# HoundThe/yara

Measured on AMD Instinct MI355X. Metric: scanned GB/s per GPU (4 GiB buffer, 10k atoms) + bit-exact match-set vs CPU, higher is better.
Workload: dtype u8; 1 GPU; config C: 10000 strings -> AC tables of stock libyara 4.2.1, 4 GiB per GPU; bytes_per_gpu=4294967296, parallelism=shard1

## Files before the change

include/yara_amd.h:

```cpp
#ifndef YARA_AMD_H
#define YARA_AMD_H

#include <stddef.h>
#include <stdint.h>

#ifdef __cplusplus
extern "C" {
#endif

#define YR_AMD_SUCCESS                0
#define YR_AMD_INSUFFICIENT_MEMORY    1
#define YR_AMD_COULD_NOT_MAP_FILE     4
#define YR_AMD_SCAN_TIMEOUT          26
#define YR_AMD_CALLBACK_ERROR        28
#define YR_AMD_INVALID_ARGUMENT      29
#define YR_AMD_INTERNAL_FATAL_ERROR  31

#define YR_AMD_MAX_ATOM_LENGTH 4

typedef struct yr_amd_tables yr_amd_tables;
typedef struct yr_amd_scanner yr_amd_scanner;

int yr_amd_tables_create(
    const uint32_t* transition_table,
// ... 42 lines not shown

int yr_amd_scan_block(
    yr_amd_scanner* scanner,
    const uint8_t* data,
    size_t size,
    const uint64_t** positions,
    uint64_t* count,
    int* all_positions);

int yr_amd_scan_device(
    yr_amd_scanner* scanner,
    const uint8_t* d_data,
    uint64_t block_size,
    uint64_t byte_begin,
    uint64_t byte_end);

int yr_amd_scan_window(
    yr_amd_scanner* scanner,
    const uint8_t* d_window,
    uint64_t window_begin,
    uint64_t window_end,
    uint64_t block_size,
    uint64_t byte_begin,
    uint64_t byte_end);

int yr_amd_scan_device_result(
    yr_amd_scanner* scanner,
    const uint64_t** d_positions,
    uint64_t* count,
    int* all_positions);

int yr_amd_scanner_set_verified_only(yr_amd_scanner* scanner, int enable);

int yr_amd_scan_device_stream_length(yr_amd_scanner* scanner, uint64_t* length);

typedef int (*yr_amd_verify_fn)(void* user, uint32_t pool_index, uint64_t offset);

int yr_amd_replay(
    const yr_amd_tables* tables,
    const uint8_t* data,
    size_t size,
    const uint64_t* positions,
    uint64_t count,
    int all_positions,
    yr_amd_verify_fn verify,
    void* user);

typedef struct
{
  uint64_t position;
  uint32_t state;
  uint32_t match;
} yr_amd_trace_rec;

int yr_amd_trace_walk(
    yr_amd_scanner* scanner,
    const uint8_t* d_data,
    size_t size,
    uint64_t data_base,
    yr_amd_trace_rec* out,
    uint64_t cap,
    uint64_t* count);

typedef struct
{
  uint32_t flags;
// ... 237 lines not shown
```

yara_amd/__init__.py:

```python
import ctypes

import numpy as np

from . import _lib
from ._lib import (CALLBACK_ERROR, COULD_NOT_MAP_FILE, INSUFFICIENT_MEMORY,
                   INTERNAL_FATAL_ERROR, INVALID_ARGUMENT, MATCH_HEX, MATCH_LITERAL,
                   MAX_ATOM_LENGTH, SCAN_TIMEOUT, SUCCESS, YaraAmdError)

__all__ = ["Tables", "Scanner", "Pipeline", "replay", "fill_xorshift64", "version",
           "batch_layout", "merge_matches", "YaraAmdError", "MATCH_LITERAL", "MATCH_HEX"]


def _arr(a, dt):
    return np.ascontiguousarray(a, dtype=dt)


def version() -> str:
    return _lib.lib().yr_amd_version().decode()


def batch_layout(sizes):
    sz = _arr(sizes, np.uint64).reshape(-1)
    st = np.zeros(sz.size, np.uint64)
    arena = ctypes.c_uint64()
# ... 466 lines not shown
    def scan_window(self, d_ptr: int, window_begin: int, window_end: int, block_size: int,
                    byte_begin: int, byte_end: int):
        _lib.check("yr_amd_scan_window",
                   _lib.lib().yr_amd_scan_window(self._h, ctypes.c_void_p(d_ptr), window_begin,
                                                 window_end, block_size, byte_begin, byte_end))

    def device_result(self):
        p = ctypes.c_void_p()
        cnt = ctypes.c_uint64()
        allp = ctypes.c_int()
        _lib.check("yr_amd_scan_device_result",
                   _lib.lib().yr_amd_scan_device_result(self._h, ctypes.byref(p), ctypes.byref(cnt),
                                                        ctypes.byref(allp)))
        return p.value or 0, cnt.value, bool(allp.value)

    def trace_walk(self, d_ptr: int, size: int, data_base: int = 0, cap=None):
        cnt = ctypes.c_uint64()
        if cap is None:
            _lib.check("yr_amd_trace_walk",
                       _lib.lib().yr_amd_trace_walk(self._h, ctypes.c_void_p(d_ptr), size, data_base,
                                                    None, 0, ctypes.byref(cnt)))
            cap = cnt.value
        out = np.zeros(cap, dtype=_lib.TRACE_REC_DTYPE)
        _lib.check("yr_amd_trace_walk",
                   _lib.lib().yr_amd_trace_walk(self._h, ctypes.c_void_p(d_ptr), size, data_base,
                                                ctypes.c_void_p(out.ctypes.data if cap else 0), cap,
                                                ctypes.byref(cnt)))
        return out[:min(cap, cnt.value)], cnt.value

    def set_verified_only(self, enable: bool = True):
        _lib.check("yr_amd_scanner_set_verified_only",
                   _lib.lib().yr_amd_scanner_set_verified_only(self._h, int(enable)))

    def stream_length(self) -> int:
        n = ctypes.c_uint64()
        _lib.check("yr_amd_scan_device_stream_length",
                   _lib.lib().yr_amd_scan_device_stream_length(self._h, ctypes.byref(n)))
        return n.value

    def set_timing(self, enable: bool = True):
        _lib.check("yr_amd_scanner_set_timing", _lib.lib().yr_amd_scanner_set_timing(self._h, int(enable)))

    def kernel_ms(self) -> float:
        ms = ctypes.c_float()
        _lib.check("yr_amd_scanner_kernel_ms", _lib.lib().yr_amd_scanner_kernel_ms(self._h, ctypes.byref(ms)))
        return ms.value

    def scan_ms(self) -> float:
        ms = ctypes.c_float()
        _lib.check("yr_amd_scanner_scan_ms", _lib.lib().yr_amd_scanner_scan_ms(self._h, ctypes.byref(ms)))
        return ms.value

    def close(self):
        if getattr(self, "_h", None):
            _lib.lib().yr_amd_scanner_destroy(self._h)
            self._h = None

    def __del__(self):
        try:
            self.close()
        except Exception:
            pass


def merge_matches(blocks):
    parts = []
# ... 139 lines not shown
```

yara_amd/_lib.py:

```python
import ctypes
import os

_HERE = os.path.dirname(os.path.abspath(__file__))
LIB_PATH = os.environ.get("YARA_AMD_LIB") or os.path.join(_HERE, "libyara_amd.so")

SUCCESS = 0
INSUFFICIENT_MEMORY = 1
COULD_NOT_MAP_FILE = 4
SCAN_TIMEOUT = 26
CALLBACK_ERROR = 28
INVALID_ARGUMENT = 29
INTERNAL_FATAL_ERROR = 31
MAX_ATOM_LENGTH = 4
MATCH_MAX_BLOCK = 1 << 32

_u32p = ctypes.POINTER(ctypes.c_uint32)
_u16p = ctypes.POINTER(ctypes.c_uint16)
_u64p = ctypes.POINTER(ctypes.c_uint64)
_u8p = ctypes.POINTER(ctypes.c_uint8)
_vp = ctypes.c_void_p
_int = ctypes.c_int

VERIFY_FN = ctypes.CFUNCTYPE(ctypes.c_int, ctypes.c_void_p, ctypes.c_uint32, ctypes.c_uint64)
COPY_FN = ctypes.CFUNCTYPE(ctypes.c_int, ctypes.c_void_p, ctypes.c_void_p, ctypes.c_void_p,
# ... 32 lines not shown
class MatchRec(ctypes.Structure):
    _fields_ = [("offset", ctypes.c_uint64), ("string", ctypes.c_uint32),
                ("length", ctypes.c_uint32), ("xor_key", ctypes.c_uint32),
                ("pool_index", ctypes.c_uint32)]


VERIFY_REC_DTYPE = [("offset", "<u8"), ("pool_index", "<u4"), ("candidate", "<u4")]
MATCH_REC_DTYPE = [("offset", "<u8"), ("string", "<u4"), ("length", "<u4"), ("xor_key", "<u4"),
                   ("pool_index", "<u4")]
TRACE_REC_DTYPE = [("position", "<u8"), ("state", "<u4"), ("match", "<u4")]

PROTOTYPES = {
    "yr_amd_tables_create": (_int, [_u32p, _u32p, ctypes.c_uint32, _u32p, _u16p, ctypes.c_uint32,
                                    _int, ctypes.POINTER(_vp)]),
    "yr_amd_tables_destroy": (_int, [_vp]),
    "yr_amd_tables_load_yarc": (_int, [_u8p, ctypes.c_size_t, _int, ctypes.POINTER(_vp)]),
    "yr_amd_tables_get_info": (_int, [_vp, ctypes.POINTER(TablesInfo)]),
    "yr_amd_scanner_create": (_int, [_vp, _vp, ctypes.POINTER(_vp)]),
    "yr_amd_scanner_destroy": (_int, [_vp]),
    "yr_amd_scan_block": (_int, [_vp, _u8p, ctypes.c_size_t, ctypes.POINTER(_u64p),
                                 ctypes.POINTER(ctypes.c_uint64), ctypes.POINTER(_int)]),
    "yr_amd_scan_device": (_int, [_vp, _vp, ctypes.c_uint64, ctypes.c_uint64, ctypes.c_uint64]),
    "yr_amd_scan_window": (_int, [_vp, _vp, ctypes.c_uint64, ctypes.c_uint64, ctypes.c_uint64,
                                  ctypes.c_uint64, ctypes.c_uint64]),
    "yr_amd_scan_device_result": (_int, [_vp, ctypes.POINTER(_vp), ctypes.POINTER(ctypes.c_uint64),
                                         ctypes.POINTER(_int)]),
    "yr_amd_replay": (_int, [_vp, _u8p, ctypes.c_size_t, _u64p, ctypes.c_uint64, _int, VERIFY_FN,
                             _vp]),
    "yr_amd_trace_walk": (_int, [_vp, _vp, ctypes.c_size_t, ctypes.c_uint64, _vp, ctypes.c_uint64,
                                 ctypes.POINTER(ctypes.c_uint64)]),
    "yr_amd_fill_xorshift64": (_int, [_vp, ctypes.c_uint64, ctypes.c_uint64, ctypes.c_uint64, _vp]),
    "yr_amd_scanner_set_timing": (_int, [_vp, _int]),
    "yr_amd_scanner_set_verified_only": (_int, [_vp, _int]),
    "yr_amd_scan_device_stream_length": (_int, [_vp, _u64p]),
    "yr_amd_scanner_kernel_ms": (_int, [_vp, ctypes.POINTER(ctypes.c_float)]),
    "yr_amd_scanner_scan_ms": (_int, [_vp, ctypes.POINTER(ctypes.c_float)]),
    "yr_amd_version": (ctypes.c_char_p, []),
    "yr_amd_tables_set_strings": (_int, [_vp, _u32p, ctypes.c_uint32, ctypes.POINTER(String),
                                         ctypes.c_uint32, _u8p, ctypes.c_uint64, _u8p]),
    "yr_amd_tables_set_re_code": (_int, [_vp, ctypes.c_uint32, _u32p, _u32p, _u32p, _u32p, _u8p,
                                         ctypes.c_uint64]),
    "yr_amd_re_code_extent": (_int, [_u8p, ctypes.c_uint64, ctypes.POINTER(ctypes.c_uint32)]),
    "yr_amd_verify_device": (_int, [_vp, ctypes.c_uint64, ctypes.POINTER(_vp),
                                    ctypes.POINTER(ctypes.c_uint64)]),
    "yr_amd_tables_final_strings": (_int, [_vp, _u8p, ctypes.c_uint32]),
    "yr_amd_tables_set_string_flags": (_int, [_vp, _u32p, ctypes.c_uint32]),
    "yr_amd_tables_string_count": (_int, [_vp, _u32p]),
    "yr_amd_match_device": (_int, [_vp, ctypes.c_uint64, ctypes.POINTER(_vp),
                                   ctypes.POINTER(ctypes.c_uint64), ctypes.POINTER(_vp),
                                   ctypes.POINTER(ctypes.c_uint64)]),
    "yr_amd_scan_block_matches": (_int, [_vp, _u8p, ctypes.c_size_t, ctypes.c_uint64,
                                         ctypes.POINTER(ctypes.POINTER(MatchRec)),
                                         ctypes.POINTER(ctypes.c_uint64),
                                         ctypes.POINTER(ctypes.POINTER(VerifyRec)),
                                         ctypes.POINTER(ctypes.c_uint64)]),
    "yr_amd_pipeline_create": (_int, [_vp, ctypes.c_uint32, ctypes.POINTER(_vp)]),
    "yr_amd_pipeline_destroy": (_int, [_vp]),
    "yr_amd_pipeline_submit": (_int, [_vp, _u8p, ctypes.c_size_t, ctypes.c_uint64]),
    "yr_amd_pipeline_submit_dma": (_int, [_vp, _u8p, ctypes.c_size_t, ctypes.c_uint64]),
    "yr_amd_pipeline_next": (_int, [_vp, ctypes.POINTER(ctypes.POINTER(VerifyRec)),
                                    ctypes.POINTER(ctypes.c_uint64), ctypes.POINTER(_u8p),
                                    ctypes.POINTER(ctypes.c_size_t), ctypes.POINTER(ctypes.c_uint64)]),
    "yr_amd_pipeline_drain": (_int, [_vp]),
    "yr_amd_pipeline_create_multi": (_int, [ctypes.POINTER(_vp), ctypes.c_uint32, ctypes.c_uint32,
                                            ctypes.POINTER(_vp)]),
    "yr_amd_pipeline_set_copy": (_int, [_vp, COPY_FN, _vp]),
# ... 72 lines not shown
```

yara_amd/csrc/internal.h:

```cpp
#pragma once

#include <stdint.h>
#include <stdlib.h>

#include <hip/hip_runtime.h>

#ifndef YAMD_DIAG
#define YAMD_DIAG 0
#endif

namespace yamd {

inline const char* diag_env(const char* name) { return YAMD_DIAG ? getenv(name) : nullptr; }

constexpr int kWave = 64;
constexpr int kBytesPerLane = 16;
constexpr int kTile = kWave * kBytesPerLane;
constexpr uint32_t kSegment = 1u << 20;
constexpr uint32_t kSegmentTarget = kSegment;
constexpr uint32_t kMaxByteKeys = 4;
constexpr uint32_t kMaxPairKeys = 4;
constexpr int kWavesPerWG = 16;
constexpr int kWGThreads = kWave * kWavesPerWG;

constexpr int kFilterLog2Bits = 20;
constexpr uint32_t kFilterWords = 1u << (kFilterLog2Bits - 5);
constexpr uint32_t kFilterBytes = kFilterWords * 4;

constexpr uint32_t kQueueCap = 64;
constexpr uint32_t kQueueEntryWords = 6;
constexpr uint32_t kQueueBytes = kWavesPerWG * kQueueCap * kQueueEntryWords * 4;
constexpr uint32_t kPendBytes = kWavesPerWG * kWave * 8;
constexpr uint32_t kScanLdsBytes = kFilterBytes + kQueueBytes + kPendBytes;

constexpr uint32_t kFilterPair = 0;
constexpr uint32_t kFilterEven = 1;
constexpr uint32_t kFilterEvenHash = 2;
constexpr uint32_t kEvenHashK = 0xEBCA77u;
struct FilterProbe {
  uint32_t block;
  uint32_t b_lo, b_hi;
};
__host__ __device__ inline FilterProbe filter_probe_left(uint32_t w3) {
  const uint32_t x = w3 & 0xFFFFFFu;
  return FilterProbe{x >> 10, x & 31u, (x >> 5) & 31u};
}
__host__ __device__ inline FilterProbe filter_probe_even(uint32_t w3, bool hashed) {
  const uint32_t x = w3 & 0xFFFFFFu;
  const uint32_t block = hashed ? (x * kEvenHashK) >> 18 : x >> 10;
  return FilterProbe{block, x & 31u, (x >> 5) & 31u};
}
__host__ __device__ inline FilterProbe filter_probe_right(uint32_t w3) {
// ... 92 lines not shown
```

yara_amd/csrc/kernels.hip:

```cpp
#include <hip/hip_ext.h>

#include "internal.h"

namespace yamd {

__device__ __forceinline__ uint32_t lane_id() {
  return __builtin_amdgcn_mbcnt_hi(~0u, __builtin_amdgcn_mbcnt_lo(~0u, 0u));
}

typedef uint32_t u32x2 __attribute__((ext_vector_type(2)));
template <typename T>
__device__ __forceinline__ T lds_load(uint32_t addr) {
  return *reinterpret_cast<const __attribute__((address_space(3))) T*>((uintptr_t)addr);
}
__device__ __forceinline__ void lds_store2(uint32_t addr, uint32_t x, uint32_t y) {
  u32x2 v;
  v.x = x;
  v.y = y;
  *reinterpret_cast<__attribute__((address_space(3))) u32x2*>((uintptr_t)addr) = v;
}

__device__ __forceinline__ uint32_t wave_inclusive_scan(uint32_t v) {
  v += __builtin_amdgcn_update_dpp(0u, v, 0x111, 0xF, 0xF, true);
  v += __builtin_amdgcn_update_dpp(0u, v, 0x112, 0xF, 0xF, true);
  v += __builtin_amdgcn_update_dpp(0u, v, 0x114, 0xF, 0xF, true);
  v += __builtin_amdgcn_update_dpp(0u, v, 0x118, 0xF, 0xF, true);
  v += __builtin_amdgcn_update_dpp(0u, v, 0x142, 0xA, 0xF, false);
  v += __builtin_amdgcn_update_dpp(0u, v, 0x143, 0xC, 0xF, false);
  return v;
}

__device__ __forceinline__ bool bucket_pair_has(const uint4& a, const uint4& b, uint32_t k) {
  const uint32_t x = min(min(a.x ^ k, a.y ^ k), a.z ^ k);
// ... 1106 lines not shown
    for (int i = 0; i < YAMD_PAD_VOP2; i += 4)
      asm volatile("v_add_u32_e32 %0, 1, %0\n v_add_u32_e32 %1, 1, %1\n v_add_u32_e32 %2, 1, %2\n v_add_u32_e32 %3, 1, %3"
                   : "+v"(t0), "+v"(t1), "+v"(t2), "+v"(t3));
#endif
#ifdef YAMD_PAD_VOP3
#pragma unroll
    for (int i = 0; i < YAMD_PAD_VOP3; i += 4)
      asm volatile("v_add3_u32 %0, %0, 1, 2\n v_add3_u32 %1, %1, 1, 2\n v_add3_u32 %2, %2, 1, 2\n v_add3_u32 %3, %3, 1, 2"
                   : "+v"(t0), "+v"(t1), "+v"(t2), "+v"(t3));
#endif
#ifdef YAMD_PAD_NOP
#pragma unroll
    for (int i = 0; i < YAMD_PAD_NOP; ++i) asm volatile("s_nop 0");
#endif
    asm volatile("" ::"v"(t0 ^ t1 ^ t2 ^ t3));
#ifdef YAMD_PAD_SALU
    uint32_t u0 = tile_off, u1 = tile_off + 1, u2 = tile_off + 2, u3 = tile_off + 3;
#pragma unroll
    for (int i = 0; i < YAMD_PAD_SALU; i += 4)
      asm volatile("s_add_u32 %0, %0, 1\n s_add_u32 %1, %1, 1\n s_add_u32 %2, %2, 1\n s_add_u32 %3, %3, 1"
                   : "+s"(u0), "+s"(u1), "+s"(u2), "+s"(u3) : : "scc");
    asm volatile("" ::"s"(u0 ^ u1 ^ u2 ^ u3));
#endif
  }
#endif
  if constexpr (kAbl<MODE> == 1) {
    asm volatile("" ::"v"(any));
  } else {
    ring_append<MODE, TAIL>(p, q, st, S, any, tile_off, lane);
  }
  if constexpr (kBkSkipF<MODE>) q.facc |= any_f;
}

template <int MODE>
__device__ __forceinline__ void scan_segment(const ScanParams& p, WaveQueue& q, uint32_t seg, uint32_t lane) {
  SegState st;
  st.seg_start = p.byte_begin + (uint64_t)seg * p.seg_bytes;
  const uint64_t seg_end = min(st.seg_start + p.seg_bytes, p.byte_end);
  st.seg_len = (uint32_t)(seg_end - st.seg_start);
  st.out = p.seg_out + (p.seg_base ? p.seg_base[seg] : (size_t)seg * p.seg_cap);
  st.found = 0;
  const uint64_t avail = p.byte_end - st.seg_start;
  const uint8_t* base = p.data + st.seg_start;

  st.carry = __builtin_amdgcn_readfirstlane(
      st.seg_start >= 4 ? *reinterpret_cast<const uint32_t*>(base - 4) : 0u);
  q.count = 0;
  q.pend_n = 0;
  q.full = 0;
  q.dacc = 0;
  q.facc = 0u;

  const uint32_t n_full = st.seg_len / kTile;
  if (n_full > 0) {
    const uint32_t full_end = n_full * kTile;
    const __amdgpu_buffer_rsrc_t rsrc = segment_rsrc(base);
    const uint32_t lane16 = lane * kBytesPerLane;
    constexpr uint32_t kP = kPf<MODE>, kR = kP + 1;
    uint4 t[kR];
#pragma unroll
    for (uint32_t i = 0; i < kP; ++i)
      if (i * kTile < full_end) t[i] = load_tile_full(rsrc, i * kTile, lane16);
    asm volatile("" : "+v"(t[0].x), "+v"(t[0].y), "+v"(t[0].z), "+v"(t[0].w));
    uint32_t off = 0;
    if (full_end >= (2 * kR - 1) * kTile) {
      const uint32_t lim = full_end - (2 * kR - 1) * kTile;
      do {
#pragma unroll
        for (uint32_t i = 0; i < kR; ++i) {
          t[(i + kP) % kR] = load_tile_full(rsrc, off + (i + kP) * kTile, lane16);
          tile_step<MODE, false>(p, q, st, t[i], off + i * kTile, lane);
        }
        off += kR * kTile;
      } while (off <= lim);
    }
    while (off < full_end) {
#pragma unroll
      for (uint32_t i = 0; i < kR; ++i) {
        if (off + i * kTile < full_end) {
          if (off + (i + kP) * kTile < full_end)
            t[(i + kP) % kR] = load_tile_full(rsrc, off + (i + kP) * kTile, lane16);
          tile_step<MODE, false>(p, q, st, t[i], off + i * kTile, lane);
        }
      }
      off += kR * kTile;
    }
  }
  if (st.seg_len % kTile != 0)
    tile_step<MODE, true>(p, q, st, load_tile(base, n_full * kTile, lane, avail), n_full * kTile,
                          lane);
  if (q.count != 0) drain<MODE>(p, q, lane, st.seg_start, st.seg_len, st.out, st.found);
  if (q.pend_n != 0) flush_pending<MODE>(p, q, lane, st.seg_start, st.out, st.found);
  if (lane == 0) {
    p.seg_count[seg] = st.found;
    if (kDrop<MODE>) p.seg_full[seg] = q.full + q.dacc;
  }
}

template <int MODE>
__global__ __launch_bounds__(kWGThreads, 1) void scan_segments_kernel(ScanParams p) {
  extern __shared__ __attribute__((aligned(16))) uint32_t lds[];
  uint32_t* filt = lds;
  {
    const uint4* src = reinterpret_cast<const uint4*>(p.filter);
    uint4* dst = reinterpret_cast<uint4*>(filt);
    constexpr uint32_t kPer = kFilterWords / 4 / kWGThreads;
    static_assert(kPer * kWGThreads * 4 == kFilterWords, "filter copy: whole uint4s per thread");
    uint4 v[kPer];
#pragma unroll
    for (uint32_t k = 0; k < kPer; ++k) v[k] = src[threadIdx.x + k * kWGThreads];
#pragma unroll
    for (uint32_t k = 0; k < kPer; ++k) dst[threadIdx.x + k * kWGThreads] = v[k];
  }
  __syncthreads();
  const uint32_t lane = lane_id();
  const uint32_t wid = __builtin_amdgcn_readfirstlane(threadIdx.x / kWave);
  const uint32_t total_waves = gridDim.x * kWavesPerWG;
  uint32_t seg = blockIdx.x * kWavesPerWG + wid;
  uint32_t kcv = 0u;
  if constexpr (kDrop<MODE>)
    if (lane < kKcWords) kcv = p.kc[lane];
  while (seg < p.n_segments) {
    WaveQueue q;
    q.kcv = kcv;
    q.ring = kFilterBytes + wid * (kQueueCap * kQueueEntryWords * 4);
    q.pend = kFilterBytes + kQueueBytes + wid * (kWave * 8);
    __builtin_amdgcn_s_setprio(1);
    scan_segment<MODE>(p, q, seg, lane);
    if (p.seg_next == nullptr) {
      seg += total_waves;
    } else {
      uint32_t t = 0;
      if (lane == 0) t = atomicAdd(p.seg_next, 1u);
      seg = __builtin_amdgcn_readfirstlane(t);
    }
  }
}

__global__ __launch_bounds__(1024) void seg_offsets_kernel(const uint32_t* seg_count, uint32_t n,
                                                           uint32_t cap, uint64_t* seg_offset,
                                                           uint64_t* summary) {
  __shared__ uint64_t wsum[kWGThreads / kWave];
  __shared__ uint32_t wmax[kWGThreads / kWave];
  const uint32_t t = threadIdx.x, lane = t % kWave, w = t / kWave;
  const uint32_t per = (n + kWGThreads - 1) / kWGThreads;
  const uint32_t lo = min(t * per, n), hi = min(lo + per, n);
  uint64_t s = 0;
  uint32_t mx = 0;
  constexpr uint32_t kKeep = 8;
  uint32_t keep[kKeep];
#pragma unroll
  for (uint32_t k = 0; k < kKeep; ++k) {
    keep[k] = lo + k < hi ? seg_count[lo + k] : 0u;
    s += min(keep[k], cap);
    mx = max(mx, keep[k]);
  }
#pragma unroll 16
  for (uint32_t i = lo + kKeep; i < hi; ++i) {
    const uint32_t c = seg_count[i];
    s += min(c, cap);
    mx = max(mx, c);
  }
  uint64_t incl = s;
  for (int d = 1; d < kWave; d <<= 1) {
    const uint64_t v = __shfl_up(incl, d, kWave);
    if (lane >= (uint32_t)d) incl += v;
  }
  for (int d = kWave / 2; d >= 1; d >>= 1) mx = max(mx, (uint32_t)__shfl_xor(mx, d, kWave));
// ... 120 lines not shown
      const bool live = valid && cls == 0u;
      const uint64_t lm = __ballot(live);
      if (lm != 0) {
        uint32_t b = 0;
        if (lane == 0) b = atomicAdd(&lcount, (uint32_t)__popcll(lm));
        b = __builtin_amdgcn_readfirstlane(b);
        const uint32_t slot =
            b + __builtin_amdgcn_mbcnt_hi((uint32_t)(lm >> 32), __builtin_amdgcn_mbcnt_lo((uint32_t)lm, 0u));
        if (live) p.live[first + slot] = (uint32_t)(first + i);
      }
    }
    {
      if (classes) {
        __syncthreads();
        const uint64_t a = first + chunk;
        const uint32_t m = cend - chunk;
        const uint32_t head = min((4u - sh0) & 3u, m);
        const uint32_t nd = (m - head) / 4u, tail = m - head - 4u * nd;
        uint8_t* out = p.dead + a;
        for (uint32_t t = threadIdx.x; t < nd; t += kStride)
          *reinterpret_cast<uint32_t*>(out + head + 4u * t) =
              *reinterpret_cast<const uint32_t*>(cbuf + sh0 + head + 4u * t);
        if (threadIdx.x < head) out[threadIdx.x] = cbuf[sh0 + threadIdx.x];
        if (threadIdx.x < tail) out[head + 4u * nd + threadIdx.x] = cbuf[sh0 + head + 4u * nd + threadIdx.x];
        __syncthreads();
      }
    }
  }
  if (!classes) return;
  __syncthreads();
  if (threadIdx.x == 0) p.live_count[seg] = lcount;
}

__global__ __launch_bounds__(256) void xorshift_fill_kernel(uint8_t* buf, uint64_t n,
                                                            const uint64_t* states,
                                                            uint32_t n_chunks, uint32_t chunk) {
  const uint32_t c = blockIdx.x * blockDim.x + threadIdx.x;
  if (c >= n_chunks) return;
  uint64_t x = states[c];
  const uint64_t lo = (uint64_t)c * chunk;
  const uint64_t hi = min(lo + chunk, n);
  uint64_t i = lo;
  for (; i + 16 <= hi; i += 16) {
    uint32_t w[4];
#pragma unroll
    for (int j = 0; j < 4; ++j) {
      uint32_t v = 0;
#pragma unroll
      for (int b = 0; b < 4; ++b) {
        x ^= x << 13;
        x ^= x >> 7;
        x ^= x << 17;
        v |= (uint32_t)((x >> 24) & 0xFF) << (8 * b);
      }
      w[j] = v;
    }
    *reinterpret_cast<uint4*>(buf + i) = make_uint4(w[0], w[1], w[2], w[3]);
  }
  for (; i < hi; ++i) {
    x ^= x << 13;
    x ^= x >> 7;
    x ^= x << 17;
    buf[i] = (uint8_t)(x >> 24);
  }
}

// ... 64 lines not shown
          YAMD_BK_CASES(kDropModes)
        } else {
          YAMD_BK_CASES(0)
        }
#undef YAMD_BK_CASES
      } else if (p.filter_mode == kFilterEven)
        YAMD_LAUNCH_SCAN(scan_segments_kernel<kModeEven>);
      else if (p.filter_mode == kFilterEvenHash)
        YAMD_LAUNCH_SCAN(scan_segments_kernel<kModeEvenHash>);
      else
        YAMD_LAUNCH_SCAN(scan_segments_kernel<0>);
      break;
  }
  return hipGetLastError();
}
#undef YAMD_LAUNCH_SCAN

hipError_t launch_compact(const ScanParams& p, uint64_t* seg_offset, uint64_t* summary,
                          uint64_t* positions, bool scatter, hipStream_t s) {
  if (!scatter) {
    hipLaunchKernelGGL(seg_offsets_kernel, dim3(1), dim3(1024), 0, s, p.seg_count, p.n_segments,
                       p.seg_cap, seg_offset, summary);
    if (p.drop_dead != 0u)
      hipLaunchKernelGGL(seg_offsets_kernel, dim3(1), dim3(1024), 0, s, (const uint32_t*)p.seg_full,
                         p.n_segments, 0xFFFFFFFFu, p.seg_full_offset, summary + 2);
  } else {
    if (p.seg_base == nullptr && p.seg_cap <= p.seg_bytes / 256)
      hipLaunchKernelGGL(seg_scatter_kernel<2>, dim3(p.n_segments), dim3(2 * kWave), 0, s, p,
                         (const uint64_t*)seg_offset, positions);
    else
      hipLaunchKernelGGL(seg_scatter_kernel<kScatterWaves>, dim3(p.n_segments), dim3(kScatterWaves * kWave),
                         0, s, p, (const uint64_t*)seg_offset, positions);
  }
  return hipGetLastError();
}

hipError_t launch_counts_offsets(const uint32_t* counts, uint32_t n, uint64_t* offsets, uint64_t* summary,
                                 hipStream_t s) {
  hipLaunchKernelGGL(seg_offsets_kernel, dim3(1), dim3(1024), 0, s, counts, n, 0xFFFFFFFFu, offsets, summary);
  return hipGetLastError();
}

hipError_t launch_xorshift(uint8_t* buf, uint64_t n, const uint64_t* states, uint32_t n_chunks,
                           uint32_t chunk, hipStream_t s) {
  hipLaunchKernelGGL(xorshift_fill_kernel, dim3((n_chunks + 255) / 256), dim3(256), 0, s, buf, n,
                     states, n_chunks, chunk);
  return hipGetLastError();
}

hipError_t configure_scan_kernel() {
  const int lds = (int)kScanLdsBytes;
  hipError_t e = hipSuccess;
  for (const void* k : {(const void*)scan_segments_kernel<0>,
                        (const void*)scan_segments_kernel<kModeByteKeys>,
                        (const void*)scan_segments_kernel<kModeByteKeysNext>,
                        (const void*)scan_segments_kernel<kModeEven>,
                        (const void*)scan_segments_kernel<kModeEvenHash>,
                        (const void*)scan_segments_kernel<kModeByteKeysEven>,
                        (const void*)scan_segments_kernel<kModeByteKeysEvenHash>,
                        (const void*)scan_segments_kernel<kModeByteKeysNextEven>,
                        (const void*)scan_segments_kernel<kModeByteKeysNextEvenHash>,
                        (const void*)scan_segments_kernel<kDropModes + kModeByteKeys>,
                        (const void*)scan_segments_kernel<kDropModes + kModeByteKeysNext>,
                        (const void*)scan_segments_kernel<kDropModes + kModeByteKeysEven>,
                        (const void*)scan_segments_kernel<kDropModes + kModeByteKeysEvenHash>,
                        (const void*)scan_segments_kernel<kDropModes + kModeByteKeysNextEven>,
// ... 38 lines not shown
```

yara_amd/csrc/scanner.cpp:

```cpp
#include <hip/hip_runtime.h>
#include <stdio.h>
#include <stdlib.h>
#include <string.h>

#include <algorithm>
#include <cmath>
#include <new>
#include <vector>

#include "../../include/yara_amd.h"
#include "internal.h"
#include "tables.h"
#include "re_program.h"
#include "verify.h"
#include "batch.h"
#include "matches.h"

namespace yamd {
hipError_t launch_scan(const ScanParams& p, int grid, hipStream_t s, int mode, hipEvent_t t0 = nullptr,
                       hipEvent_t t1 = nullptr);
hipError_t launch_compact(const ScanParams& p, uint64_t* seg_offset, uint64_t* summary,
                          uint64_t* positions, bool scatter, hipStream_t s);
hipError_t launch_xorshift(uint8_t* buf, uint64_t n, const uint64_t* states, uint32_t n_chunks,
                           uint32_t chunk, hipStream_t s);
hipError_t configure_scan_kernel();
hipError_t launch_trace_count(const uint32_t* T, const uint8_t* data, uint64_t n_pos,
                              uint32_t* block_count, uint32_t n_blocks, hipStream_t s);
hipError_t launch_trace_write(const uint32_t* T, const uint32_t* M, const uint8_t* data,
                              uint64_t n_pos, const uint64_t* block_offset,
                              yr_amd_trace_rec* out, uint64_t cap, uint32_t n_blocks,
                              hipStream_t s);
}

namespace yamd {
uint32_t re_general_extent(const uint8_t* c, uint64_t avail) {
  const uint64_t lim = std::min<uint64_t>(avail, 1u << 20);
  if (lim == 0) return 0;
  std::vector<uint8_t> seen(lim, 0);
  std::vector<int64_t> work{0};
  uint64_t end = 0;
  while (!work.empty()) {
    int64_t ip = work.back();
    work.pop_back();
    while (true) {
      if (ip < 0 || (uint64_t)ip >= lim) return 0;
      if (seen[ip]) break;
      seen[ip] = 1;
      const uint8_t op = c[ip];
      const uint32_t sz = re_op_size(op);
      if (sz == 0 || (uint64_t)ip + sz > lim) return 0;
      end = std::max<uint64_t>(end, (uint64_t)ip + sz);
      if (op == kOpMatch) break;
      if (op == kOpJump) {
        ip += re_i16(c + ip + 1);
        continue;
// ... 74 lines not shown
  uint32_t* d_seg_full = nullptr;
  uint64_t* d_seg_full_offset = nullptr;
  uint32_t* d_cand_index = nullptr;
  size_t cand_index_cap = 0;
  uint64_t last_full_count = 0;
  size_t positions_cap = 0;
  uint64_t* h_summary = nullptr;
  uint64_t* d_hsum = nullptr;
  uint64_t* d_summary = nullptr;

  std::vector<uint64_t> h_positions;

  uint32_t* d_trace_T = nullptr;
  uint32_t* d_trace_M = nullptr;

  ScanParams last{};
  uint64_t win_lo = 0, win_hi = 0;
  int last_grid = 0;
  bool last_all = false;
  bool last_empty = false;
  bool pending = false;
  uint64_t last_count = 0;

  bool timing = false;
  hipEvent_t ev_begin = nullptr, ev_end = nullptr, ev_compact = nullptr;
  hipEvent_t ev_done = nullptr;
  hipEvent_t last_done = nullptr;
  hipEvent_t ev_counted = nullptr;
  hipEvent_t last_counted = nullptr;
  bool ev_valid = false;

  int diag_mode = 0;
  uint32_t dense_per_kib = 0;
  uint64_t* d_seg_base = nullptr;
  uint32_t* d_seg_next = nullptr;
  size_t seg_base_cap = 0;
  uint64_t rerun_total = 0;

  uint32_t* d_vcount = nullptr;
  size_t vcount_cap = 0;
  uint32_t* d_vkeep = nullptr;
  size_t vkeep_cap = 0;
  uint64_t* d_vblock = nullptr;
  uint64_t* d_vchunk = nullptr;
  size_t vchunk_cap = 0;
  size_t vblock_cap = 0;
  VerifyRec* d_vrec = nullptr;
  size_t vrec_cap = 0;
  std::vector<yr_amd_verify_rec> h_vrec;

  bool scanned = false;
  uint64_t* d_mkeys = nullptr;
  uint32_t* d_mindex = nullptr;
  MatchMeasure* d_mmeas = nullptr;
  VerifyRec* d_mrest = nullptr;
  MatchRec* d_mout = nullptr;
  size_t match_cap = 0;
  uint64_t* d_mblock = nullptr;
  size_t mblock_cap = 0;
  uint64_t* d_mchunk = nullptr;
  size_t mchunk_cap = 0;
  uint64_t* d_mhist = nullptr;
  size_t mhist_cap = 0;
  uint64_t* d_mhchunk = nullptr;
  size_t mhchunk_cap = 0;
  uint64_t* h_msum = nullptr;
// ... 107 lines not shown
  return grow(s->d_seg_out, s->seg_out_cap, (size_t)n_segments * seg_cap);
}

uint32_t choose_seg_bytes(uint64_t nbytes, int num_cus, uint32_t target) {
  const uint64_t waves = (uint64_t)num_cus * kWavesPerWG;
  const uint64_t k = std::max<uint64_t>(1, (nbytes + waves * target - 1) / (waves * target));
  uint64_t per = (nbytes + waves * k - 1) / (waves * k);
  per = (per + kTile - 1) / kTile * kTile;
  return (uint32_t)std::min<uint64_t>(std::max<uint64_t>(per, 4 * kTile), kSegment);
}

int run_scan(yr_amd_scanner* s) {
  const ScanParams& p = s->last;
  const size_t out_cap = p.seg_base ? s->rerun_total : (size_t)p.n_segments * p.seg_cap;
  int r = grow(s->d_positions, s->positions_cap, out_cap);
  if (!r && s->tables->kd_any) r = grow(s->d_dead, s->dead_cap, out_cap);
  if (!r && s->tables->kd_any) r = grow(s->d_live, s->live_cap, out_cap);
  if (!r && s->tables->kd_any) r = grow(s->d_seg_x, s->seg_x_cap, out_cap);
  if (!r && p.drop_dead) r = grow(s->d_cand_index, s->cand_index_cap, out_cap);
  if (r) return r;
  s->last.dead = s->tables->kd_any ? s->d_dead : nullptr;
  s->last.live = s->tables->kd_any ? s->d_live : nullptr;
  s->last.live_count = s->tables->kd_any ? s->d_live_count : nullptr;
  s->last.seg_x = s->tables->kd_any ? s->d_seg_x : nullptr;
  s->last.seg_full = p.drop_dead ? s->d_seg_full : nullptr;
  s->last.seg_full_offset = p.drop_dead ? s->d_seg_full_offset : nullptr;
  s->last.cand_index = p.drop_dead ? s->d_cand_index : nullptr;
  if (s->timing) {
    HIP_TRY(launch_scan(p, s->last_grid, s->stream, s->diag_mode, s->ev_begin, s->ev_end));
    s->ev_valid = true;
  } else {
    HIP_TRY(launch_scan(p, s->last_grid, s->stream, s->diag_mode));
  }
  HIP_TRY(launch_compact(p, s->d_seg_offset, s->d_hsum, nullptr, false, s->stream));
  s->last_counted = nullptr;
  if (s->verified_only) {
    HIP_TRY(hipEventRecord(s->ev_counted, s->stream));
    s->last_counted = s->ev_counted;
  }
  HIP_TRY(launch_compact(p, s->d_seg_offset, s->d_hsum, s->d_positions, true, s->stream));
  s->last_done = s->timing ? s->ev_compact : s->ev_done;
  HIP_TRY(hipEventRecord(s->last_done, s->stream));
  return YR_AMD_SUCCESS;
}

}

extern "C" {

const char* yr_amd_version(void) { return "yara_amd 0.1.0 (gfx950)"; }

int yr_amd_tables_create(const uint32_t* transition_table, const uint32_t* match_table,
                         uint32_t n_slots, const uint32_t* pool_next,
                         const uint16_t* pool_backtrack, uint32_t n_pool, int device,
                         yr_amd_tables** tables) {
  if (tables == nullptr) return YR_AMD_INVALID_ARGUMENT;
  *tables = nullptr;
  yr_amd_tables* t = new (std::nothrow) yr_amd_tables();
  if (t == nullptr) return YR_AMD_INSUFFICIENT_MEMORY;
  int r = flatten_tables(transition_table, match_table, n_slots, pool_next, pool_backtrack, n_pool,
                         t->flat);
  if (r != YR_AMD_SUCCESS) {
    delete t;
    return r;
  }
  t->device = device;
  if (device < 0) {
    *tables = t;
    return YR_AMD_SUCCESS;
  }
  if (hipSetDevice(device) != hipSuccess ||
      hipDeviceGetAttribute(&t->num_cus, hipDeviceAttributeMultiprocessorCount, device) !=
          hipSuccess ||
// ... 95 lines not shown
                  (void*)s->d_seg_offset,
                  (void*)s->d_seg_out, (void*)s->d_positions, (void*)s->d_dead, (void*)s->d_live,
                  (void*)s->d_seg_x, (void*)s->d_seg_full, (void*)s->d_seg_full_offset,
                  (void*)s->d_cand_index, (void*)s->d_live_count, (void*)s->d_live_off,
                  (void*)s->d_summary,
                  (void*)s->d_vcount, (void*)s->d_vkeep, (void*)s->d_vblock, (void*)s->d_vrec,
                  (void*)s->d_vchunk, (void*)s->d_seg_base,
                  (void*)s->d_seg_next, (void*)s->d_trace_T, (void*)s->d_trace_M,
                  (void*)s->d_bstarts, (void*)s->d_boff, (void*)s->d_btmp, (void*)s->d_bpos,
                  (void*)s->d_bunit, (void*)s->d_bunit_off, (void*)s->d_gather,
                  (void*)s->d_mkeys, (void*)s->d_mindex, (void*)s->d_mmeas, (void*)s->d_mrest,
                  (void*)s->d_mout, (void*)s->d_mblock, (void*)s->d_mchunk, (void*)s->d_mhist,
                  (void*)s->d_mhchunk, (void*)s->d_mbuf, (void*)s->d_moff, (void*)s->d_hkeys,
                  (void*)s->d_hmeas, (void*)s->d_hsets, (void*)s->d_hrest, (void*)s->d_hblock,
                  (void*)s->d_hchunk})
    if (p) (void)hipFree(p);
  if (s->h_msum) (void)hipHostFree(s->h_msum);
  if (s->h_arena) (void)hipHostFree(s->h_arena);
  if (s->h_summary) (void)hipHostFree(s->h_summary);
  if (s->ev_begin) (void)hipEventDestroy(s->ev_begin);
  if (s->ev_end) (void)hipEventDestroy(s->ev_end);
  if (s->ev_compact) (void)hipEventDestroy(s->ev_compact);
  if (s->ev_done) (void)hipEventDestroy(s->ev_done);
  if (s->ev_counted) (void)hipEventDestroy(s->ev_counted);
  if (s->ev_gather) (void)hipEventDestroy(s->ev_gather);
  if (s->own_stream && s->stream) (void)hipStreamDestroy(s->stream);
  delete s;
  return YR_AMD_SUCCESS;
}

int yr_amd_scanner_set_verified_only(yr_amd_scanner* s, int enable) {
  if (s == nullptr) return YR_AMD_INVALID_ARGUMENT;
  s->verified_only = enable != 0;
  return YR_AMD_SUCCESS;
}

int yr_amd_scan_device_stream_length(yr_amd_scanner* s, uint64_t* length) {
  if (s == nullptr || length == nullptr || s->pending) return YR_AMD_INVALID_ARGUMENT;
  *length = s->last_full_count;
  return YR_AMD_SUCCESS;
}

int yr_amd_scanner_set_timing(yr_amd_scanner* s, int enable) {
  if (s == nullptr) return YR_AMD_INVALID_ARGUMENT;
  if (enable && s->ev_begin == nullptr) {
    HIP_TRY(hipSetDevice(s->tables->device));
    const unsigned marker = hipEventDisableSystemFence;
    HIP_TRY(hipEventCreateWithFlags(&s->ev_begin, marker));
    HIP_TRY(hipEventCreateWithFlags(&s->ev_end, marker));
    HIP_TRY(hipEventCreate(&s->ev_compact));
  }
  s->timing = enable != 0;
  s->ev_valid = false;
  return YR_AMD_SUCCESS;
}

#if YAMD_DIAG
int64_t yr_amd__diag_dead_count(yr_amd_scanner* s) {
  if (s == nullptr || s->last.dead == nullptr || s->last_count == 0) return -1;
  std::vector<uint8_t> h(s->last_count);
  if (hipMemcpy(h.data(), s->last.dead, h.size(), hipMemcpyDeviceToHost) != hipSuccess) return -2;
  int64_t n = 0;
  for (uint8_t x : h) n += x != 0;
  return n;
}

// ... 57 lines not shown
  s->batch_done = false;
  s->last_count = 0;
  s->last_full_count = 0;
  s->ev_valid = false;
  s->win_lo = window_begin;
  s->win_hi = window_end;
  const uint8_t* d_data =
      d_window == nullptr ? nullptr : (const uint8_t*)((uintptr_t)d_window - (uintptr_t)window_begin);
  s->last.data = d_data;
  s->last.block_size = block_size;
  s->last.byte_begin = byte_begin;
  s->last.byte_end = byte_end;
  s->last_all = t->flat.root_accepting;
  s->last_empty = s->last_all || byte_end == byte_begin;
  s->last.dead = nullptr;
  s->last.live = nullptr;
  s->last.live_count = nullptr;
  s->last.seg_x = nullptr;
  s->last.drop_dead = 0;
  s->last.seg_full = nullptr;
  s->last.seg_full_offset = nullptr;
  s->last.cand_index = nullptr;
  if (s->last_empty) return YR_AMD_SUCCESS;
  if (d_window == nullptr) return YR_AMD_INVALID_ARGUMENT;
  HIP_TRY(hipSetDevice(t->device));

  const uint64_t nbytes = byte_end - byte_begin;
  static const uint32_t seg_target = [] {
    const char* e = diag_env("YAMD_SEG_KIB");
    const uint32_t k = e ? (uint32_t)atoi(e) : 0u;
    return k >= 4 && k * 1024u <= kSegment ? k * 1024u : kSegmentTarget;
  }();
  static const bool dynamic = diag_env("YAMD_SEG_DYNAMIC") != nullptr;
  const uint32_t seg_bytes = choose_seg_bytes(nbytes, t->num_cus, seg_target);
  const uint64_t n_segments64 = (nbytes + seg_bytes - 1) / seg_bytes;
  if (n_segments64 > 0xFFFFFFFFull) return YR_AMD_INVALID_ARGUMENT;
  const uint32_t n_segments = (uint32_t)n_segments64;
  const uint32_t learned = (uint32_t)std::min<uint64_t>(
      (uint64_t)s->dense_per_kib * seg_bytes / 1024, seg_bytes / 64);
  const uint32_t seg_cap = std::max<uint32_t>(std::max<uint32_t>(64, seg_bytes / 256), learned);
  int r = ensure_segments(s, n_segments, seg_cap);
  if (r) return r;

  ScanParams& p = s->last;
  p.data = d_data;
  p.block_size = block_size;
  p.byte_begin = byte_begin;
  p.byte_end = byte_end;
  p.filter = t->d_filter;
  p.exact = t->d_exact;
  p.t3_off = t->flat.t3_off;
  p.t3_mask = t->flat.t3_mask;
  p.t4_off = t->flat.t4_off;
  p.t4_mask = t->flat.t4_mask;
  p.exact_flags = t->flat.exact_flags;
  p.len_mask = t->flat.len_mask;
  p.byte_keys = t->flat.byte_keys;
  p.n_byte_keys = t->flat.n_byte_keys;
  p.pair_keys[0] = t->flat.pair_keys[0];
  p.pair_keys[1] = t->flat.pair_keys[1];
  p.n_pair_keys = t->flat.n_pair_keys;
  p.kx_end = t->kx_end;
  p.kx_deep = t->kx_deep;
  p.kx_next = t->kx_next;
  for (int k = 0; k < 4; ++k) {
    p.kd_m[k] = t->kd_m[k];
    p.kd_v[k] = t->kd_v[k];
// ... 1665 lines not shown
```

Before: 5265 GB/s.

## Prefetch next segment's tiles during drain and fuse two-pass compaction

Result: slower. 5182 GB/s (-1.6%).

```diff
diff --git a/include/yara_amd.h b/include/yara_amd.h
--- a/include/yara_amd.h
+++ b/include/yara_amd.h
@@ -98,6 +98,8 @@
 
 int yr_amd_scanner_set_verified_only(yr_amd_scanner* scanner, int enable);
 
+int yr_amd_scanner_set_segment_target(yr_amd_scanner* scanner, uint32_t bytes);
+
 int yr_amd_scan_device_stream_length(yr_amd_scanner* scanner, uint64_t* length);
 
 typedef int (*yr_amd_verify_fn)(void* user, uint32_t pool_index, uint64_t offset);
diff --git a/yara_amd/__init__.py b/yara_amd/__init__.py
--- a/yara_amd/__init__.py
+++ b/yara_amd/__init__.py
@@ -522,6 +522,10 @@
         _lib.check("yr_amd_scanner_set_verified_only",
                    _lib.lib().yr_amd_scanner_set_verified_only(self._h, int(enable)))
 
+    def set_segment_target(self, nbytes: int = 0):
+        _lib.check("yr_amd_scanner_set_segment_target",
+                   _lib.lib().yr_amd_scanner_set_segment_target(self._h, int(nbytes)))
+
     def stream_length(self) -> int:
         n = ctypes.c_uint64()
         _lib.check("yr_amd_scan_device_stream_length",
diff --git a/yara_amd/_lib.py b/yara_amd/_lib.py
--- a/yara_amd/_lib.py
+++ b/yara_amd/_lib.py
@@ -88,6 +88,7 @@
     "yr_amd_fill_xorshift64": (_int, [_vp, ctypes.c_uint64, ctypes.c_uint64, ctypes.c_uint64, _vp]),
     "yr_amd_scanner_set_timing": (_int, [_vp, _int]),
     "yr_amd_scanner_set_verified_only": (_int, [_vp, _int]),
+    "yr_amd_scanner_set_segment_target": (_int, [_vp, ctypes.c_uint32]),
     "yr_amd_scan_device_stream_length": (_int, [_vp, _u64p]),
     "yr_amd_scanner_kernel_ms": (_int, [_vp, ctypes.POINTER(ctypes.c_float)]),
     "yr_amd_scanner_scan_ms": (_int, [_vp, ctypes.POINTER(ctypes.c_float)]),
diff --git a/yara_amd/csrc/internal.h b/yara_amd/csrc/internal.h
--- a/yara_amd/csrc/internal.h
+++ b/yara_amd/csrc/internal.h
@@ -18,6 +18,10 @@
 constexpr int kTile = kWave * kBytesPerLane;
 constexpr uint32_t kSegment = 1u << 20;
 constexpr uint32_t kSegmentTarget = kSegment;
+#ifndef YAMD_FUSED_MAX_SEGMENTS
+#define YAMD_FUSED_MAX_SEGMENTS 8192
+#endif
+constexpr uint32_t kFusedMaxSegments = YAMD_FUSED_MAX_SEGMENTS;
 constexpr uint32_t kMaxByteKeys = 4;
 constexpr uint32_t kMaxPairKeys = 4;
 constexpr int kWavesPerWG = 16;
diff --git a/yara_amd/csrc/kernels.hip b/yara_amd/csrc/kernels.hip
--- a/yara_amd/csrc/kernels.hip
+++ b/yara_amd/csrc/kernels.hip
@@ -1,4 +1,6 @@
 #include <hip/hip_ext.h>
+
+#include <algorithm>
 
 #include "internal.h"
 
@@ -1171,8 +1173,53 @@
   if constexpr (kBkSkipF<MODE>) q.facc |= any_f;
 }
 
-template <int MODE>
-__device__ __forceinline__ void scan_segment(const ScanParams& p, WaveQueue& q, uint32_t seg, uint32_t lane) {
+#ifdef YAMD_NO_SEG_AHEAD
+template <int MODE>
+constexpr bool kSegAhead = false;
+#else
+template <int MODE>
+constexpr bool kSegAhead = !kDrop<MODE>;
+#endif
+template <int MODE>
+struct SegHead {
+  uint32_t halo;
+  uint4 t[kPf<MODE> + 1];
+};
+
+__device__ __forceinline__ uint32_t load_halo(const uint8_t* base, uint64_t seg_start) {
+  return seg_start >= 4 ? *reinterpret_cast<const uint32_t*>(base - 4) : 0u;
+}
+template <int MODE>
+__device__ __forceinline__ void request_tiles(SegHead<MODE>& h, __amdgpu_buffer_rsrc_t rsrc,
+                                              uint32_t full_end, uint32_t lane16) {
+#pragma unroll
+  for (uint32_t i = 0; i < kPf<MODE>; ++i)
+    if (i * kTile < full_end) h.t[i] = load_tile_full(rsrc, i * kTile, lane16);
+}
+template <int MODE>
+__device__ __forceinline__ void segment_request(const ScanParams& p, uint32_t seg, uint32_t lane,
+                                                SegHead<MODE>& h) {
+  const uint64_t seg_start = p.byte_begin + (uint64_t)seg * p.seg_bytes;
+  const uint64_t seg_end = min(seg_start + p.seg_bytes, p.byte_end);
+  const uint8_t* base = p.data + seg_start;
+  h.halo = load_halo(base, seg_start);
+  request_tiles<MODE>(h, segment_rsrc(base), (uint32_t)(seg_end - seg_start) / kTile * kTile,
+                      lane * kBytesPerLane);
+}
+
+__device__ __forceinline__ uint32_t next_segment(const ScanParams& p, uint32_t seg, uint32_t total_waves,
+                                                 uint32_t lane) {
+  if (p.seg_next == nullptr) return seg + total_waves;
+  uint32_t t = 0;
+  if (lane == 0) t = atomicAdd(p.seg_next, 1u);
+  return __builtin_amdgcn_readfirstlane(t);
+}
+
+template <int MODE>
+__device__ __forceinline__ uint32_t scan_segment(const ScanParams& p, WaveQueue& q, uint32_t seg, uint32_t lane,
+                                                 uint32_t total_waves, SegHead<MODE>& ahead) {
+  SegHead<MODE> own;
+  SegHead<MODE>& h = *(kSegAhead<MODE> ? &ahead : &own);
   SegState st;
   st.seg_start = p.byte_begin + (uint64_t)seg * p.seg_bytes;
   const uint64_t seg_end = min(st.seg_start + p.seg_bytes, p.byte_end);
@@ -1182,8 +1229,8 @@
   const uint64_t avail = p.byte_end - st.seg_start;
   const uint8_t* base = p.data + st.seg_start;
 
-  st.carry = __builtin_amdgcn_readfirstlane(
-      st.seg_start >= 4 ? *reinterpret_cast<const uint32_t*>(base - 4) : 0u);
+  if constexpr (!kSegAhead<MODE>) h.halo = load_halo(base, st.seg_start);
+  st.carry = __builtin_amdgcn_readfirstlane(h.halo);
   q.count = 0;
   q.pend_n = 0;
   q.full = 0;
@@ -1196,10 +1243,8 @@
     const __amdgpu_buffer_rsrc_t rsrc = segment_rsrc(base);
     const uint32_t lane16 = lane * kBytesPerLane;
     constexpr uint32_t kP = kPf<MODE>, kR = kP + 1;
-    uint4 t[kR];
-#pragma unroll
-    for (uint32_t i = 0; i < kP; ++i)
-      if (i * kTile < full_end) t[i] = load_tile_full(rsrc, i * kTile, lane16);
+    uint4 (&t)[kR] = h.t;
+    if constexpr (!kSegAhead<MODE>) request_tiles<MODE>(h, rsrc, full_end, lane16);
     asm volatile("" : "+v"(t[0].x), "+v"(t[0].y), "+v"(t[0].z), "+v"(t[0].w));
     uint32_t off = 0;
     if (full_end >= (2 * kR - 1) * kTile) {
@@ -1228,18 +1273,32 @@
   if (st.seg_len % kTile != 0)
     tile_step<MODE, true>(p, q, st, load_tile(base, n_full * kTile, lane, avail), n_full * kTile,
                           lane);
+  uint32_t next = 0;
+  if constexpr (kSegAhead<MODE>) {
+    next = next_segment(p, seg, total_waves, lane);
+    if (next < p.n_segments) segment_request<MODE>(p, next, lane, h);
+  }
   if (q.count != 0) drain<MODE>(p, q, lane, st.seg_start, st.seg_len, st.out, st.found);
   if (q.pend_n != 0) flush_pending<MODE>(p, q, lane, st.seg_start, st.out, st.found);
   if (lane == 0) {
     p.seg_count[seg] = st.found;
     if (kDrop<MODE>) p.seg_full[seg] = q.full + q.dacc;
   }
+  if constexpr (!kSegAhead<MODE>) next = next_segment(p, seg, total_waves, lane);
+  return next;
 }
 
 template <int MODE>
 __global__ __launch_bounds__(kWGThreads, 1) void scan_segments_kernel(ScanParams p) {
   extern __shared__ __attribute__((aligned(16))) uint32_t lds[];
   uint32_t* filt = lds;
+  const uint32_t lane = lane_id();
+  const uint32_t wid = __builtin_amdgcn_readfirstlane(threadIdx.x / kWave);
+  const uint32_t total_waves = gridDim.x * kWavesPerWG;
+  uint32_t seg = blockIdx.x * kWavesPerWG + wid;
+  SegHead<MODE> h;
+  if constexpr (kSegAhead<MODE>)
+    if (seg < p.n_segments) segment_request<MODE>(p, seg, lane, h);
   {
     const uint4* src = reinterpret_cast<const uint4*>(p.filter);
     uint4* dst = reinterpret_cast<uint4*>(filt);
@@ -1252,10 +1311,6 @@
     for (uint32_t k = 0; k < kPer; ++k) dst[threadIdx.x + k * kWGThreads] = v[k];
   }
   __syncthreads();
-  const uint32_t lane = lane_id();
-  const uint32_t wid = __builtin_amdgcn_readfirstlane(threadIdx.x / kWave);
-  const uint32_t total_waves = gridDim.x * kWavesPerWG;
-  uint32_t seg = blockIdx.x * kWavesPerWG + wid;
   uint32_t kcv = 0u;
   if constexpr (kDrop<MODE>)
     if (lane < kKcWords) kcv = p.kc[lane];
@@ -1265,14 +1320,7 @@
     q.ring = kFilterBytes + wid * (kQueueCap * kQueueEntryWords * 4);
     q.pend = kFilterBytes + kQueueBytes + wid * (kWave * 8);
     __builtin_amdgcn_s_setprio(1);
-    scan_segment<MODE>(p, q, seg, lane);
-    if (p.seg_next == nullptr) {
-      seg += total_waves;
-    } else {
-      uint32_t t = 0;
-      if (lane == 0) t = atomicAdd(p.seg_next, 1u);
-      seg = __builtin_amdgcn_readfirstlane(t);
-    }
+    seg = scan_segment<MODE>(p, q, seg, lane, total_waves, h);
   }
 }
 
@@ -1459,6 +1507,72 @@
   if (threadIdx.x == 0) p.live_count[seg] = lcount;
 }
 
+constexpr uint32_t kFusedThreads = 256;
+__global__ __launch_bounds__(kFusedThreads) void seg_compact_kernel(
+    const uint32_t* seg_count, const uint32_t* seg_out, uint32_t n, uint32_t cap, uint32_t seg_bytes,
+    uint64_t byte_begin, uint32_t group, uint64_t* seg_offset, uint64_t* summary, uint64_t* positions) {
+  constexpr uint32_t kWaves = kFusedThreads / kWave;
+  __shared__ uint64_t wsum[kWaves], wtot[kWaves];
+  __shared__ uint32_t wmax[kWaves];
+  const uint32_t t = threadIdx.x, lane = t % kWave, w = t / kWave;
+  const uint32_t seg0 = blockIdx.x * group;
+  const uint32_t seg1 = min(seg0 + group, n);
+  const bool last = seg1 == n;
+  uint32_t e = 0;
+  if (t < cap) e = seg_out[(size_t)seg0 * cap + t];
+  const uint32_t hi = last ? n : seg0;
+  uint64_t s = 0, tot = 0;
+  uint32_t mx = 0;
+#pragma unroll 16
+  for (uint32_t i = t; i < hi; i += kFusedThreads) {
+    const uint32_t c = seg_count[i];
+    const uint32_t v = min(c, cap);
+    s += i < seg0 ? v : 0u;
+    tot += v;
+    mx = max(mx, c);
+  }
+  for (int d = kWave / 2; d >= 1; d >>= 1) {
+    s += __shfl_xor(s, d, kWave);
+    tot += __shfl_xor(tot, d, kWave);
+    mx = max(mx, (uint32_t)__shfl_xor(mx, d, kWave));
+  }
+  if (lane == 0) {
+    wsum[w] = s;
+    wtot[w] = tot;
+    wmax[w] = mx;
+  }
+  __syncthreads();
+  uint64_t run = 0;
+#pragma unroll
+  for (uint32_t k = 0; k < kWaves; ++k) run += wsum[k];
+  if (last && t == 0) {
+    uint64_t all = 0;
+    uint32_t m = 0;
+#pragma unroll
+    for (uint32_t k = 0; k < kWaves; ++k) {
+      all += wtot[k];
+      m = max(m, wmax[k]);
+    }
+    __hip_atomic_store(&summary[0], all, __ATOMIC_RELAXED, __HIP_MEMORY_SCOPE_SYSTEM);
+    __hip_atomic_store(&summary[1], (uint64_t)m, __ATOMIC_RELAXED, __HIP_MEMORY_SCOPE_SYSTEM);
+    seg_offset[n] = all;
+  }
+  for (uint32_t seg = seg0; seg < seg1; ++seg) {
+    const uint32_t c = min(seg_count[seg], cap);
+    if (t == 0) seg_offset[seg] = run;
+    const uint64_t base = byte_begin + (uint64_t)seg * seg_bytes + 1;
+    const uint32_t* src = seg_out + (size_t)seg * cap;
+    uint64_t* dst = positions + run;
+    for (uint32_t i = t; i < c; i += kFusedThreads) {
+      const uint32_t ec = e;
+      if (i + kFusedThreads < c) e = src[i + kFusedThreads];
+      __builtin_nontemporal_store(base + (ec & kOutOffsetMask), dst + i);
+    }
+    if (seg + 1 < seg1 && t < cap) e = src[cap + t];
+    run += c;
+  }
+}
+
 __global__ __launch_bounds__(256) void xorshift_fill_kernel(uint8_t* buf, uint64_t n,
                                                             const uint64_t* states,
                                                             uint32_t n_chunks, uint32_t chunk) {
@@ -1589,6 +1703,21 @@
       hipLaunchKernelGGL(seg_scatter_kernel<kScatterWaves>, dim3(p.n_segments), dim3(kScatterWaves * kWave),
                          0, s, p, (const uint64_t*)seg_offset, positions);
   }
+  return hipGetLastError();
+}
+
+bool compact_is_fused(const ScanParams& p) {
+  static const bool off = diag_env("YAMD_NO_FUSED_COMPACT") != nullptr;
+  return !off && p.dead == nullptr && p.drop_dead == 0u && p.seg_base == nullptr &&
+         p.seg_cap <= std::max(64u, p.seg_bytes / 256) && p.n_segments <= kFusedMaxSegments;
+}
+
+hipError_t launch_compact_fused(const ScanParams& p, uint64_t* seg_offset, uint64_t* summary,
+                                uint64_t* positions, hipStream_t s) {
+  const uint32_t group = std::min(std::max(kSegment / p.seg_bytes, 1u), 8u);
+  hipLaunchKernelGGL(seg_compact_kernel, dim3((p.n_segments + group - 1) / group), dim3(kFusedThreads),
+                     0, s, (const uint32_t*)p.seg_count, (const uint32_t*)p.seg_out, p.n_segments,
+                     p.seg_cap, p.seg_bytes, p.byte_begin, group, seg_offset, summary, positions);
   return hipGetLastError();
 }
 
diff --git a/yara_amd/csrc/scanner.cpp b/yara_amd/csrc/scanner.cpp
--- a/yara_amd/csrc/scanner.cpp
+++ b/yara_amd/csrc/scanner.cpp
@@ -21,6 +21,9 @@
                        hipEvent_t t1 = nullptr);
 hipError_t launch_compact(const ScanParams& p, uint64_t* seg_offset, uint64_t* summary,
                           uint64_t* positions, bool scatter, hipStream_t s);
+bool compact_is_fused(const ScanParams& p);
+hipError_t launch_compact_fused(const ScanParams& p, uint64_t* seg_offset, uint64_t* summary,
+                                uint64_t* positions, hipStream_t s);
 hipError_t launch_xorshift(uint8_t* buf, uint64_t n, const uint64_t* states, uint32_t n_chunks,
                            uint32_t chunk, hipStream_t s);
 hipError_t configure_scan_kernel();
@@ -161,6 +164,7 @@
 
   int diag_mode = 0;
   uint32_t dense_per_kib = 0;
+  uint32_t seg_target = 0;
   uint64_t* d_seg_base = nullptr;
   uint32_t* d_seg_next = nullptr;
   size_t seg_base_cap = 0;
@@ -334,13 +338,17 @@
   } else {
     HIP_TRY(launch_scan(p, s->last_grid, s->stream, s->diag_mode));
   }
-  HIP_TRY(launch_compact(p, s->d_seg_offset, s->d_hsum, nullptr, false, s->stream));
   s->last_counted = nullptr;
-  if (s->verified_only) {
-    HIP_TRY(hipEventRecord(s->ev_counted, s->stream));
-    s->last_counted = s->ev_counted;
-  }
-  HIP_TRY(launch_compact(p, s->d_seg_offset, s->d_hsum, s->d_positions, true, s->stream));
+  if (!s->verified_only && compact_is_fused(p)) {
+    HIP_TRY(launch_compact_fused(p, s->d_seg_offset, s->d_hsum, s->d_positions, s->stream));
+  } else {
+    HIP_TRY(launch_compact(p, s->d_seg_offset, s->d_hsum, nullptr, false, s->stream));
+    if (s->verified_only) {
+      HIP_TRY(hipEventRecord(s->ev_counted, s->stream));
+      s->last_counted = s->ev_counted;
+    }
+    HIP_TRY(launch_compact(p, s->d_seg_offset, s->d_hsum, s->d_positions, true, s->stream));
+  }
   s->last_done = s->timing ? s->ev_compact : s->ev_done;
   HIP_TRY(hipEventRecord(s->last_done, s->stream));
   return YR_AMD_SUCCESS;
@@ -502,6 +510,14 @@
 int yr_amd_scanner_set_verified_only(yr_amd_scanner* s, int enable) {
   if (s == nullptr) return YR_AMD_INVALID_ARGUMENT;
   s->verified_only = enable != 0;
+  return YR_AMD_SUCCESS;
+}
+
+int yr_amd_scanner_set_segment_target(yr_amd_scanner* s, uint32_t bytes) {
+  if (s == nullptr) return YR_AMD_INVALID_ARGUMENT;
+  const uint64_t tiles = ((uint64_t)bytes + kTile - 1) / kTile;
+  s->seg_target = bytes == 0 ? 0u
+                             : (uint32_t)std::min<uint64_t>(std::max<uint64_t>(tiles, 4) * kTile, kSegment);
   return YR_AMD_SUCCESS;
 }
 
@@ -625,7 +641,8 @@
     return k >= 4 && k * 1024u <= kSegment ? k * 1024u : kSegmentTarget;
   }();
   static const bool dynamic = diag_env("YAMD_SEG_DYNAMIC") != nullptr;
-  const uint32_t seg_bytes = choose_seg_bytes(nbytes, t->num_cus, seg_target);
+  const uint32_t seg_bytes =
+      choose_seg_bytes(nbytes, t->num_cus, s->seg_target != 0 ? s->seg_target : seg_target);
   const uint64_t n_segments64 = (nbytes + seg_bytes - 1) / seg_bytes;
   if (n_segments64 > 0xFFFFFFFFull) return YR_AMD_INVALID_ARGUMENT;
   const uint32_t n_segments = (uint32_t)n_segments64;
```
